# aleflabo/PREGO

Measured on AMD Instinct MI355X. Metric: frames/sec (per-frame action logits) on Assembly101-O TSN features, higher is better.
Workload: dtype fp16; 1 GPU; BASELINE configs[1]: Assembly101-O-test-split-shaped eval set, MiniROAD eval path (rgb+flow fp32 [T,2048] each -> per-frame probs[86] + argmax); clips_per_gpu=182, frames_per_gpu=2306143, min_T=3342, max_T=33981, flow=non-zero (full K=4096 layer1 GEMM), parallelism=clip-sharded dp1, no collective: every rank its own eval-set-sized clip list, weights=random init, seed 20

## Files before the change

prego_amd/csrc/ff_pass.hip:

```cpp
#include "common.h"
#include "kernels.h"
#include "pass_handshake.h"

#define FBK 64
#define FHALF 16384
#define FBUF 65536
#define FF_WAIT(n) asm volatile("s_waitcnt vmcnt(" #n ")" ::: "memory")
#define FF_TIMEOUT_TICKS 200000000ull

__device__ __forceinline__ int ffp_key_b(int r) { return ((r >> 1) & 1) | (((r >> 3) & 3) << 1); }

__device__ __forceinline__ bool ffp_wait_ge(const unsigned* p, unsigned need, unsigned* abort_word, unsigned code) {
  if (__hip_atomic_load(p, __ATOMIC_RELAXED, __HIP_MEMORY_SCOPE_AGENT) >= need) return true;
  const unsigned long long t0 = __builtin_amdgcn_s_memrealtime();
  unsigned spins = 0;
  for (;;) {
    __builtin_amdgcn_s_sleep(8);
    if (__hip_atomic_load(p, __ATOMIC_RELAXED, __HIP_MEMORY_SCOPE_AGENT) >= need) return true;
    if ((++spins & 31u) == 0u) {
      if (__hip_atomic_load(abort_word, __ATOMIC_RELAXED, __HIP_MEMORY_SCOPE_AGENT)) return false;
      if (__builtin_amdgcn_s_memrealtime() - t0 > FF_TIMEOUT_TICKS) {
        __hip_atomic_store(abort_word, code, __ATOMIC_RELAXED, __HIP_MEMORY_SCOPE_AGENT);
        return false;
      }
    }
  }
}

template <typename OT, bool SC1OUT>
__device__ __forceinline__ void ffp_tile(char* smem, const bf16_t* __restrict__ A, int lda, int rows, const bf16_t* __restrict__ B, int ldb,
                                         const float* __restrict__ bias, bf16_t* __restrict__ C, int ldc, int K) {
  int tid = threadIdx.x;
  asm volatile("" : "+v"(tid));
  const int lane = tid & 63;
  const int wave = __builtin_amdgcn_readfirstlane(tid >> 6);
  const int grp = wave >> 2, wc = wave & 3;
  const int nk = K / FBK;
  const int sr = lane >> 3, scp = lane & 7;
  int a_off[2], b_off[2];
#pragma unroll
  for (int i = 0; i < 2; ++i) {
    const int r = (wave * 2 + i) * 8 + sr;
    a_off[i] = r * lda * 2 + ((scp ^ ((r >> 1) & 7)) << 4);
    b_off[i] = r * ldb * 2 + ((scp ^ ffp_key_b(r)) << 4);
  }
  const __amdgpu_buffer_rsrc_t rs_a = __builtin_amdgcn_make_buffer_rsrc((void*)A, 0, rows * lda * 2, 0x00020000);
  const __amdgpu_buffer_rsrc_t rs_b = __builtin_amdgcn_make_buffer_rsrc((void*)B, 0, 256 * ldb * 2, 0x00020000);
  auto stage_a = [&](int hf, int kt) {
    char* dst = smem + (kt & 1) * FBUF + hf * FHALF + wave * 2048;
    const int so = hf * 128 * lda * 2 + kt * (FBK * 2);
#pragma unroll
    for (int i = 0; i < 2; ++i)
      __builtin_amdgcn_raw_ptr_buffer_load_lds(rs_a, (__attribute__((address_space(3))) void*)(dst + i * 1024), 16, a_off[i], so, 0, 0);
  };
  auto stage_b = [&](int hf, int kt) {
    char* dst = smem + (kt & 1) * FBUF + (2 + hf) * FHALF + wave * 2048;
    const int so = hf * 128 * ldb * 2 + kt * (FBK * 2);
#pragma unroll
    for (int i = 0; i < 2; ++i)
      __builtin_amdgcn_raw_ptr_buffer_load_lds(rs_b, (__attribute__((address_space(3))) void*)(dst + i * 1024), 16, b_off[i], so, 0, 0);
  };
  const int fr = lane & 15, fq = lane >> 4;
  bf16x8 a0[2][4], a1[2][4], b0[2][2], b1[2][2];
  auto read_a = [&](bf16x8 (&af)[2][4], int slot, int kt) {
    const char* base = smem + (kt & 1) * FBUF + slot * FHALF;
#pragma unroll
    for (int ks = 0; ks < 2; ++ks)
#pragma unroll
      for (int i = 0; i < 4; ++i) {
        const int r = grp * 64 + i * 16 + fr;
        af[ks][i] = *(const bf16x8*)(base + r * 128 + (((ks * 4 + fq) ^ ((r >> 1) & 7)) << 4));
      }
  };
  auto read_b = [&](bf16x8 (&bf)[2][2], int slot, int kt) {
    const char* base = smem + (kt & 1) * FBUF + slot * FHALF;
#pragma unroll
    for (int ks = 0; ks < 2; ++ks)
#pragma unroll
      for (int j = 0; j < 2; ++j) {
        const int r = wc * 32 + (fr >> 2) * 8 + j * 4 + (fr & 3);
        bf[ks][j] = *(const bf16x8*)(base + r * 128 + (((ks * 4 + fq) ^ ffp_key_b(r)) << 4));
      }
  };
  f32x4 acc[2][2][4][2];
#pragma unroll
  for (int x = 0; x < 2; ++x)
#pragma unroll
    for (int y = 0; y < 2; ++y)
#pragma unroll
      for (int i = 0; i < 4; ++i)
#pragma unroll
        for (int j = 0; j < 2; ++j) acc[x][y][i][j] = (f32x4){0.f, 0.f, 0.f, 0.f};
  auto mma = [&](f32x4 (&c)[4][2], const bf16x8 (&af)[2][4], const bf16x8 (&bf)[2][2]) {
    asm volatile("s_waitcnt lgkmcnt(0)" ::: "memory");
    __builtin_amdgcn_sched_barrier(0);
    __builtin_amdgcn_s_setprio(1);
#pragma unroll
    for (int ks = 0; ks < 2; ++ks)
#pragma unroll
      for (int i = 0; i < 4; ++i)
#pragma unroll
        for (int j = 0; j < 2; ++j) c[i][j] = op16<OT>::mfma(bf[ks][j], af[ks][i], c[i][j]);
    __builtin_amdgcn_s_setprio(0);
    __builtin_amdgcn_sched_barrier(0);
  };
  auto bar = [&]() {
    __builtin_amdgcn_sched_barrier(0);
    __builtin_amdgcn_s_barrier();
    __builtin_amdgcn_sched_barrier(0);
  };
  stage_a(0, 0); stage_b(0, 0); stage_b(1, 0); stage_a(1, 0);
  stage_a(0, 1); stage_b(0, 1); stage_b(1, 1);
  FF_WAIT(10);
  bar();
  read_a(a0, 0, 0);
  if (grp == 1) bar();
  for (int kt = 0; kt < nk; ++kt) {
    const bool full = kt + 2 < nk;
    read_b(b0, 2, kt);
    if (kt + 1 < nk) stage_a(1, kt + 1);
    if (full) FF_WAIT(10); else FF_WAIT(0);
    bar();
    mma(acc[0][0], a0, b0);
    bar();
    read_b(b1, 3, kt);
    if (full) { stage_a(0, kt + 2); FF_WAIT(10); } else FF_WAIT(0);
    bar();
    mma(acc[0][1], a0, b1);
    bar();
    read_a(a1, 1, kt);
    if (full) { stage_b(0, kt + 2); FF_WAIT(10); } else FF_WAIT(0);
    bar();
    mma(acc[1][1], a1, b1);
    bar();
    if (kt + 1 < nk) read_a(a0, 0, kt + 1);
    if (full) { stage_b(1, kt + 2); FF_WAIT(10); } else FF_WAIT(0);
    bar();
    mma(acc[1][0], a1, b0);
    bar();
  }
  if (grp == 0) bar();
  float4 bv[2][2];
#pragma unroll
  for (int y = 0; y < 2; ++y)
#pragma unroll
    for (int j = 0; j < 2; ++j) bv[y][j] = *(const float4*)(bias + y * 128 + wc * 32 + fq * 8 + j * 4);
  const __amdgpu_buffer_rsrc_t rs_c = __builtin_amdgcn_make_buffer_rsrc((void*)C, 0, rows * ldc * 2, 0x00020000);
#pragma unroll
  for (int x = 0; x < 2; ++x)
#pragma unroll
    for (int y = 0; y < 2; ++y) {
      const int n = y * 128 + wc * 32 + fq * 8;
#pragma unroll
      for (int i = 0; i < 4; ++i) {
        const int m = x * 128 + grp * 64 + i * 16 + fr;
        const f32x4 v0 = acc[x][y][i][0], v1 = acc[x][y][i][1];
        u32x4 pk;
        pk[0] = op16<OT>::pack2_sat(v0[0] + bv[y][0].x, v0[1] + bv[y][0].y); pk[1] = op16<OT>::pack2_sat(v0[2] + bv[y][0].z, v0[3] + bv[y][0].w);
        pk[2] = op16<OT>::pack2_sat(v1[0] + bv[y][1].x, v1[1] + bv[y][1].y); pk[3] = op16<OT>::pack2_sat(v1[2] + bv[y][1].z, v1[3] + bv[y][1].w);
        if constexpr (SC1OUT) __builtin_amdgcn_raw_buffer_store_b128(pk, rs_c, (m * ldc + n) * 2, 0, AUX_SC1);
        else __builtin_amdgcn_raw_buffer_store_b128(pk, rs_c, (m * ldc + n) * 2, 0, 0);
      }
    }
}

template <typename OT, bool IN16>
__device__ __forceinline__ void ffp_pack_rows(const FfPassArgs& a, int my_rows, int wave, int lane, const char* srgb, const char* sflow,
                                              bf16_t* __restrict__ Xs) {
  constexpr int ES = IN16 ? 2 : 4, NV = IN16 ? 1 : 2;
  constexpr int PR = 2;
  const int din = a.kx;
  const int cr_rgb = (a.d_rgb + 2047) >> 11, cpr = cr_rgb + ((a.d_flow + 2047) >> 11);
  const int n_rounds = my_rows > 0 ? ((my_rows + PR - 1) / PR) * cpr : 0;
  auto readlane_ptr = [](const char* p, int l) -> const char* {
    const unsigned long long v = (unsigned long long)p;
    const unsigned lo = (unsigned)__builtin_amdgcn_readlane((int)(unsigned)v, l), hi = (unsigned)__builtin_amdgcn_readlane((int)(unsigned)(v >> 32), l);
    return (const char*)(((unsigned long long)hi << 32) | lo);
  };
  int voff_in = lane * 8 * ES, voff_in2 = voff_in + 1024 * ES, voff_out = lane * 16;
  asm volatile("" : "+v"(voff_in), "+v"(voff_in2), "+v"(voff_out));
  auto issue = [&](u32x4 (&v)[PR][4][NV], int k) {
    const int rp = k / cpr, cj = k - rp * cpr;
    const bool fl = cj >= cr_rgb;
    const int cwin = (fl ? cj - cr_rgb : cj) << 11, seg_len = fl ? a.d_flow : a.d_rgb;
#pragma unroll
    for (int e = 0; e < PR; ++e) {
      const int r = rp * PR + e, rr = r < my_rows ? r : 0;
      const char* s0 = readlane_ptr(srgb, rr);
      const char* s1 = readlane_ptr(sflow, rr);
      const char* src = fl ? s1 : s0;
      const __amdgpu_buffer_rsrc_t rs = __builtin_amdgcn_make_buffer_rsrc((void*)(src + (size_t)cwin * ES), 0,
                                                                          (r < my_rows && src != nullptr) ? (seg_len - cwin) * ES : 0, 0x00020000);
#pragma unroll
      for (int b = 0; b < 4; ++b)
#pragma unroll
        for (int w = 0; w < NV; ++w)
          v[e][b][w] = __builtin_amdgcn_raw_buffer_load_b128(rs, (b < 2 ? voff_in : voff_in2) + ((b & 1) * 512 * ES + 16 * w), 0, AUX_NT);
    }
  };
  auto drain = [&](const u32x4 (&v)[PR][4][NV], int k) {
    const int rp = k / cpr, cj = k - rp * cpr;
    const bool fl = cj >= cr_rgb;
    const int cwin = (fl ? cj - cr_rgb : cj) << 11, seg_len = fl ? a.d_flow : a.d_rgb, seg_base = fl ? a.d_rgb : 0;
#pragma unroll
    for (int e = 0; e < PR; ++e) {
      const int r = rp * PR + e;
      bf16_t* dst = Xs + (size_t)(wave * 32 + (r < my_rows ? r : 0)) * din + seg_base + cwin;
      const __amdgpu_buffer_rsrc_t rs = __builtin_amdgcn_make_buffer_rsrc((void*)dst, 0, r < my_rows ? (seg_len - cwin) * 2 : 0, 0x00020000);
#pragma unroll
      for (int b = 0; b < 4; ++b) {
        u32x4 o = v[e][b][0];
        if constexpr (!IN16) {
          const u32x4 x = v[e][b][0], y = v[e][b][NV - 1];
          o[0] = op16<OT>::pack2_sat(__uint_as_float(x[0]), __uint_as_float(x[1])); o[1] = op16<OT>::pack2_sat(__uint_as_float(x[2]), __uint_as_float(x[3]));
          o[2] = op16<OT>::pack2_sat(__uint_as_float(y[0]), __uint_as_float(y[1])); o[3] = op16<OT>::pack2_sat(__uint_as_float(y[2]), __uint_as_float(y[3]));
        }
        __builtin_amdgcn_raw_buffer_store_b128(o, rs, voff_out + b * 1024, 0, 0);
      }
    }
  };
  u32x4 va[PR][4][NV], vb[PR][4][NV];
  if (n_rounds == 0) return;
  issue(va, 0);
  int k = 0;
#define PACK_FENCE() __builtin_amdgcn_sched_barrier(0)
  for (; k + 2 < n_rounds; k += 2) {
    issue(vb, k + 1); PACK_FENCE();
    drain(va, k); PACK_FENCE();
    issue(va, k + 2); PACK_FENCE();
    drain(vb, k + 1); PACK_FENCE();
  }
  if (k + 1 < n_rounds) {
    issue(vb, k + 1); PACK_FENCE();
    drain(va, k); PACK_FENCE();
    drain(vb, k + 1);
  } else {
    drain(va, k);
  }
#undef PACK_FENCE
}

template <typename OT>
__device__ __forceinline__ void ffp_pack(const FfPassArgs& a, int row0, int nrows, bf16_t* __restrict__ Xs) {
  int tid_ = threadIdx.x;
  asm volatile("" : "+v"(tid_));
  const int lane = tid_ & 63, wave = __builtin_amdgcn_readfirstlane(tid_ >> 6);
  const int rl = wave * 32 + (lane & 31);
  int clip = 0, t = 0;
  if (rl < nrows) {
    const int row = row0 + rl;
    int lo = a.plan.blk_step[row >> 5];
    while (lo + 1 < a.plan.s_max && a.plan.rowoff[lo + 1] <= row) ++lo;
    const int slot = row - a.plan.rowoff[lo];
    int k = a.plan.seg_off[slot];
    const int kend = a.plan.seg_off[slot + 1];
    while (k + 1 < kend && a.plan.seg_start[k + 1] <= lo) ++k;
    clip = a.plan.seg_clip[k];
    t = lo - a.plan.seg_start[k];
    if (a.rowmap != nullptr && lane < 32) ((int2*)a.rowmap)[row] = make_int2(clip, t);
  }
  const char* srgb = nullptr; const char* sflow = nullptr;
  const int es = a.in16 ? 2 : 4;
  if (rl < nrows) {
    const float* rgb = a.rgb_ptrs ? a.rgb_ptrs[clip] : nullptr;
    const float* flow = a.flow_ptrs ? a.flow_ptrs[clip] : nullptr;
    if (rgb) srgb = (const char*)rgb + (size_t)t * a.d_rgb * es;
    if (flow) sflow = (const char*)flow + (size_t)t * a.d_flow * es;
  }
  const int my_rows = nrows - wave * 32 < 32 ? nrows - wave * 32 : 32;
  if (a.in16) ffp_pack_rows<OT, true>(a, my_rows, wave, lane, srgb, sflow, Xs);
  else ffp_pack_rows<OT, false>(a, my_rows, wave, lane, srgb, sflow, Xs);
}

constexpr int FLN_MAX_E = 2048;

template <typename OT, int NV, int NR>
__device__ __forceinline__ void ffp_ln(const FfPassArgs& a, int nrows, const bf16_t* __restrict__ Ys, bf16_t* __restrict__ Es, const float* gb) {
  int tid_ = threadIdx.x;
  asm volatile("" : "+v"(tid_));
  const int lane = tid_ & 63, wave = __builtin_amdgcn_readfirstlane(tid_ >> 6);
  const int E = NV * 512;
  const float fE = (float)a.E;
  if (wave >= nrows) return;
  auto request = [&](u32x4 (&dst)[NR][NV], int rb) {
#pragma unroll
    for (int e = 0; e < NR; ++e) {
      int r = rb + 8 * e;
      if (r >= nrows) r = wave;
      const bf16_t* y = Ys + (size_t)r * E;
#pragma unroll
      for (int i = 0; i < NV; ++i) dst[e][i] = *(const u32x4*)(y + (i * 64 + lane) * 8);
    }
  };
  auto unpack = [](const u32x4 w, float (&f)[8]) {
    f[0] = op16<OT>::lo(w[0]); f[1] = op16<OT>::hi(w[0]); f[2] = op16<OT>::lo(w[1]); f[3] = op16<OT>::hi(w[1]);
    f[4] = op16<OT>::lo(w[2]); f[5] = op16<OT>::hi(w[2]); f[6] = op16<OT>::lo(w[3]); f[7] = op16<OT>::hi(w[3]);
  };
  auto process = [&](const u32x4 (&raw)[NR][NV], int rb) {
    float s[NR];
#pragma unroll
    for (int e = 0; e < NR; ++e) {
      s[e] = 0.f;
#pragma unroll
      for (int i = 0; i < NV; ++i) {
        float f[8];
        unpack(raw[e][i], f);
        s[e] += ((f[0] + f[1]) + (f[2] + f[3])) + ((f[4] + f[5]) + (f[6] + f[7]));
      }
    }
    auto wave_sum_rows = [](float (&v)[NR]) {
#pragma unroll
      for (int o = 32; o > 0; o >>= 1) {
        float t[NR];
#pragma unroll
        for (int e = 0; e < NR; ++e) t[e] = __shfl_xor(v[e], o, 64);
#pragma unroll
        for (int e = 0; e < NR; ++e) v[e] += t[e];
      }
    };
    float mu[NR], rstd[NR];
    wave_sum_rows(s);
#pragma unroll
    for (int e = 0; e < NR; ++e) mu[e] = s[e] / fE;
#pragma unroll
    for (int e = 0; e < NR; ++e) {
      float qq = 0.f;
#pragma unroll
      for (int i = 0; i < NV; ++i) {
        float f[8];
        unpack(raw[e][i], f);
#pragma unroll
        for (int k = 0; k < 8; ++k) {
#pragma clang fp contract(off)
          const float d = f[k] - mu[e];
          const float dd = d * d;
          qq = qq + dd;
        }
      }
      rstd[e] = qq;
    }
    wave_sum_rows(rstd);
#pragma unroll
    for (int e = 0; e < NR; ++e) rstd[e] = 1.0f / sqrtf(rstd[e] / fE + a.ln_eps);
#pragma unroll
    for (int i = 0; i < NV; ++i) {
      const int c = (i * 64 + lane) * 8;
      const float4 g0 = *(const float4*)(gb + c), g1 = *(const float4*)(gb + c + 4);
      const float4 b0 = *(const float4*)(gb + FLN_MAX_E + c), b1 = *(const float4*)(gb + FLN_MAX_E + c + 4);
      const float gg[8] = {g0.x, g0.y, g0.z, g0.w, g1.x, g1.y, g1.z, g1.w};
      const float bb[8] = {b0.x, b0.y, b0.z, b0.w, b1.x, b1.y, b1.z, b1.w};
#pragma unroll
      for (int e = 0; e < NR; ++e) {
        float f[8], o[8];
        unpack(raw[e][i], f);
#pragma unroll
        for (int k = 0; k < 8; ++k) o[k] = fmaxf((f[k] - mu[e]) * rstd[e] * gg[k] + bb[k], 0.f);
        uint4 w;
        w.x = op16<OT>::pack2_sat(o[0], o[1]); w.y = op16<OT>::pack2_sat(o[2], o[3]); w.z = op16<OT>::pack2_sat(o[4], o[5]); w.w = op16<OT>::pack2_sat(o[6], o[7]);
        if (rb + 8 * e < nrows) *(uint4*)(Es + (size_t)(rb + 8 * e) * E + c) = w;
      }
    }
  };
  constexpr int STEP = 8 * NR;
#define LN_FENCE() __builtin_amdgcn_sched_barrier(0)
  u32x4 ra[NR][NV], rbuf[NR][NV];
  int rb = wave;
  request(ra, rb); LN_FENCE();
  for (; rb + 2 * STEP < nrows; rb += 2 * STEP) {
    request(rbuf, rb + STEP); LN_FENCE();
    process(ra, rb); LN_FENCE();
    request(ra, rb + 2 * STEP); LN_FENCE();
    process(rbuf, rb + STEP); LN_FENCE();
  }
  if (rb + STEP < nrows) {
    request(rbuf, rb + STEP); LN_FENCE();
    process(ra, rb); LN_FENCE();
    process(rbuf, rb + STEP);
  } else {
    process(ra, rb);
  }
#undef LN_FENCE
}

template <typename OT, int MAXV, int NR>
__device__ __forceinline__ void ffp_ln_generic(const FfPassArgs& a, int nrows, const bf16_t* __restrict__ Ys, bf16_t* __restrict__ Es) {
  int tid_ = threadIdx.x;
  asm volatile("" : "+v"(tid_));
  const int lane = tid_ & 63, wave = tid_ >> 6;
  const int E = a.E, nv = E / 512;
  u32x4 raw[NR][MAXV], nxt[NR][MAXV];
  auto request = [&](u32x4 (&dst)[NR][MAXV], int rb) {
#pragma unroll
    for (int e = 0; e < NR; ++e) {
      int r = rb + 8 * e;
      if (r >= nrows) r = wave < nrows ? wave : 0;
      const bf16_t* y = Ys + (size_t)r * E;
#pragma unroll
      for (int i = 0; i < MAXV; ++i)
        if (i < nv) dst[e][i] = *(const u32x4*)(y + (i * 64 + lane) * 8);
    }
  };
  if (wave < nrows) request(raw, wave);
  for (int rb = wave; rb < nrows; rb += 8 * NR) {
    if (rb + 8 * NR < nrows) request(nxt, rb + 8 * NR);
    auto unpack = [](const u32x4 w, float (&f)[8]) {
      f[0] = op16<OT>::lo(w[0]); f[1] = op16<OT>::hi(w[0]); f[2] = op16<OT>::lo(w[1]); f[3] = op16<OT>::hi(w[1]);
      f[4] = op16<OT>::lo(w[2]); f[5] = op16<OT>::hi(w[2]); f[6] = op16<OT>::lo(w[3]); f[7] = op16<OT>::hi(w[3]);
    };
    float s[NR];
#pragma unroll
    for (int e = 0; e < NR; ++e) {
      s[e] = 0.f;
#pragma unroll
      for (int i = 0; i < MAXV; ++i)
        if (i < nv) {
          float f[8];
          unpack(raw[e][i], f);
          s[e] += ((f[0] + f[1]) + (f[2] + f[3])) + ((f[4] + f[5]) + (f[6] + f[7]));
        }
    }
    float mu[NR], rstd[NR];
#pragma unroll
    for (int e = 0; e < NR; ++e) mu[e] = wave_sum(s[e]) / (float)E;
#pragma unroll
    for (int e = 0; e < NR; ++e) {
      float qq = 0.f;
#pragma unroll
      for (int i = 0; i < MAXV; ++i)
        if (i < nv) {
          float f[8];
          unpack(raw[e][i], f);
#pragma unroll
          for (int k = 0; k < 8; ++k) {
#pragma clang fp contract(off)
            const float d = f[k] - mu[e];
            const float dd = d * d;
            qq = qq + dd;
          }
        }
      rstd[e] = qq;
    }
#pragma unroll
    for (int e = 0; e < NR; ++e) rstd[e] = 1.0f / sqrtf(wave_sum(rstd[e]) / (float)E + a.ln_eps);
#pragma unroll
    for (int i = 0; i < MAXV; ++i)
      if (i < nv) {
        const int c = (i * 64 + lane) * 8;
        const float4 g0 = *(const float4*)(a.ln_g + c), g1 = *(const float4*)(a.ln_g + c + 4);
        const float4 b0 = *(const float4*)(a.ln_b + c), b1 = *(const float4*)(a.ln_b + c + 4);
        const float gg[8] = {g0.x, g0.y, g0.z, g0.w, g1.x, g1.y, g1.z, g1.w};
        const float bb[8] = {b0.x, b0.y, b0.z, b0.w, b1.x, b1.y, b1.z, b1.w};
#pragma unroll
        for (int e = 0; e < NR; ++e) {
          float f[8], o[8];
          unpack(raw[e][i], f);
#pragma unroll
          for (int k = 0; k < 8; ++k) o[k] = fmaxf((f[k] - mu[e]) * rstd[e] * gg[k] + bb[k], 0.f);
          uint4 w;
          w.x = op16<OT>::pack2_sat(o[0], o[1]); w.y = op16<OT>::pack2_sat(o[2], o[3]); w.z = op16<OT>::pack2_sat(o[4], o[5]); w.w = op16<OT>::pack2_sat(o[6], o[7]);
          if (rb + 8 * e < nrows) *(uint4*)(Es + (size_t)(rb + 8 * e) * E + c) = w;
        }
      }
    if (rb + 8 * NR < nrows) {
#pragma unroll
      for (int e = 0; e < NR; ++e)
#pragma unroll
        for (int i = 0; i < MAXV; ++i)
          if (i < nv) raw[e][i] = nxt[e][i];
    }
  }
}

template <typename OT>
__device__ __forceinline__ void ffp_ln_any(const FfPassArgs& a, int nrows, const bf16_t* __restrict__ Ys, bf16_t* __restrict__ Es, const float* gb) {
  switch (a.E >> 9) {
    case 4: ffp_ln<OT, 4, 2>(a, nrows, Ys, Es, gb); break;
    case 2: ffp_ln<OT, 2, 4>(a, nrows, Ys, Es, gb); break;
    case 1: ffp_ln<OT, 1, 4>(a, nrows, Ys, Es, gb); break;
    default: ffp_ln_generic<OT, 8, 2>(a, nrows, Ys, Es); break;
  }
}

template <typename OT>
__global__ __launch_bounds__(512, 2) void ff_pass_kernel(FfPassArgs a) {
  extern __shared__ __attribute__((aligned(16))) char smem[];
  __shared__ int s_job[2];
  const int tid = threadIdx.x;
  const int xcc = __builtin_amdgcn_readfirstlane(__builtin_amdgcn_s_getreg((3 << 11) | 20) & 7);
  if (xcc < a.xcd_lo) return;
  if (tid == 0) {
    const unsigned nth = __hip_atomic_fetch_add(a.hs.ff_here + xcc, 1u, __ATOMIC_RELAXED, __HIP_MEMORY_SCOPE_AGENT);
    s_job[1] = hs_wait(a.hs, a.hs.ticks_all) == PREGO_HS_GO ? 1 : 0;
    if (a.max_wg > 0 && (int)nth >= a.max_wg) s_job[1] = 0;
  }
  __syncthreads();
  if (!__builtin_amdgcn_readfirstlane(s_job[1])) return;
  __shared__ __attribute__((aligned(16))) float s_gb[2 * FLN_MAX_E];
  if (a.E <= FLN_MAX_E)
    for (int c = tid; c < a.E; c += 512) { s_gb[c] = a.ln_g[c]; s_gb[FLN_MAX_E + c] = a.ln_b[c]; }
  const int q = xcc - a.xcd_lo, nf = 8 - a.xcd_lo;
  const int n_q = a.n_units > q ? (a.n_units - q + nf - 1) / nf : 0;
  const int sg = a.sg, tpr = sg * (2 + a.nt1 + a.nt2);
  const int n_rounds = (n_q + sg - 1) / sg + a.lag3;
  __shared__ unsigned long long s_stat[11];
  const bool stats = a.stats != nullptr && tid == 0;
  if (stats) {
    for (int e = 0; e < 8; ++e) s_stat[e] = 0;
    s_stat[9] = __builtin_amdgcn_s_memrealtime(); s_stat[8] = s_stat[9]; s_stat[10] = __builtin_amdgcn_s_memtime();
  }
#define FSTAT(i) do { if (stats) { const unsigned long long n_ = __builtin_amdgcn_s_memrealtime(); s_stat[i] += n_ - s_stat[8]; s_stat[8] = n_; } } while (0)
  for (;;) {
    __syncthreads();
    if (tid == 0) s_job[0] = (int)__hip_atomic_fetch_add(a.tick + q, 1u, __ATOMIC_RELAXED, __HIP_MEMORY_SCOPE_AGENT);
    __syncthreads();
    const int k = __builtin_amdgcn_readfirstlane(s_job[0]);
    const int round = k / tpr, j = k - round * tpr;
    FSTAT(5);
    if (round >= n_rounds) break;
    int type, i, nb = 0;
    if (j < sg) { type = 0; i = round * sg + j; }
    else if (j < sg + sg * a.nt1) { const int jj = j - sg; type = 1; nb = jj / sg; i = (round - a.lag1) * sg + (jj - nb * sg); }
    else if (j < 2 * sg + sg * a.nt1) { type = 2; i = (round - a.lag2) * sg + (j - sg - sg * a.nt1); }
    else { const int jj = j - 2 * sg - sg * a.nt1; type = 3; nb = jj / sg; i = (round - a.lag3) * sg + (jj - nb * sg); }
    if (i < 0 || i >= n_q) continue;
    const int u = q + i * nf;
    if (tid == 0) {
      bool ok = true;
      const int up = u - a.ring_units;
      if (type == 0) {
        if (up >= 0) ok = ffp_wait_ge(a.l1_cnt + up, (unsigned)a.nt1, a.abort_word, 0x100u);
      } else if (type == 1) {
        ok = ffp_wait_ge(a.pack_done + u, 1u, a.abort_word, 0x101u);
        if (ok && up >= 0) ok = ffp_wait_ge(a.ln_done + up, 1u, a.abort_word, 0x102u);
      } else if (type == 2) {
        ok = ffp_wait_ge(a.l1_cnt + u, (unsigned)a.nt1, a.abort_word, 0x103u);
        if (ok && up >= 0) ok = ffp_wait_ge(a.wih_cnt + up, (unsigned)a.nt2, a.abort_word, 0x104u);
      } else {
        ok = ffp_wait_ge(a.ln_done + u, 1u, a.abort_word, 0x105u);
        const int ug = u - a.gi_ring_units;
        if (ok && ug >= 0) ok = ffp_wait_ge(a.rec_cnt + (ug >> a.chunk_unit_shift), (unsigned)a.rec_expect, a.abort_word, 0x106u);
      }
      s_job[1] = ok ? 1 : 0;
    }
    __syncthreads();
    if (!__builtin_amdgcn_readfirstlane(s_job[1])) break;
    FSTAT(4);
    asm volatile("buffer_inv sc0" ::: "memory");
    const int row0 = u * 256;
    const int nrows = a.total_rows - row0 < 256 ? a.total_rows - row0 : 256;
    const size_t slot = (size_t)(u % a.ring_units) * 256;
    if (type == 0) {
      if (!(a.dbg & 1)) ffp_pack<OT>(a, row0, nrows, a.X + slot * a.kx);
    } else if (type == 1) {
      if (!(a.dbg & 4))
      ffp_tile<OT, false>(smem, a.X + slot * a.kx, a.kx, nrows, a.w1 + (size_t)nb * 256 * a.ld_w1, a.ld_w1, a.b1 + nb * 256,
                          a.Y + slot * a.E + nb * 256, a.E, a.kx);
    } else if (type == 2) {
      if (a.dbg & 2) { }
      else ffp_ln_any<OT>(a, nrows, a.Y + slot * a.E, a.Eb + slot * a.E, s_gb);
    } else {
      const size_t gslot = (size_t)(u & (a.gi_ring_units - 1)) * 256;
      if (!(a.dbg & 8))
      ffp_tile<OT, true>(smem, a.Eb + slot * a.E, a.E, nrows, a.w_ih + (size_t)nb * 256 * a.E, a.E, a.bias2 + nb * 256,
                         a.GI + gslot * a.n3 + nb * 256, a.n3, a.E);
    }
    asm volatile("s_waitcnt vmcnt(0)" ::: "memory");
    __syncthreads();
    FSTAT(type);
    if (tid == 0) {
      if (type == 0) __hip_atomic_store(a.pack_done + u, 1u, __ATOMIC_RELAXED, __HIP_MEMORY_SCOPE_AGENT);
      else if (type == 1) __hip_atomic_fetch_add(a.l1_cnt + u, 1u, __ATOMIC_RELAXED, __HIP_MEMORY_SCOPE_AGENT);
      else if (type == 2) __hip_atomic_store(a.ln_done + u, 1u, __ATOMIC_RELAXED, __HIP_MEMORY_SCOPE_AGENT);
      else {
        const unsigned old = __hip_atomic_fetch_add(a.wih_cnt + u, 1u, __ATOMIC_RELAXED, __HIP_MEMORY_SCOPE_AGENT);
        if (old + 1u == (unsigned)a.nt2)
          __hip_atomic_fetch_add(a.gi_cnt + (u >> a.chunk_unit_shift), 1u, __ATOMIC_RELAXED, __HIP_MEMORY_SCOPE_AGENT);
      }
    }
  }
  if (stats) {
    s_stat[7] = __builtin_amdgcn_s_memrealtime() - s_stat[9];
    s_stat[6] = __builtin_amdgcn_s_memtime() - s_stat[10];
    for (int e = 0; e < 8; ++e) atomicAdd(a.stats + e, s_stat[e]);
  }
#undef FSTAT
}

int launch_ff_pass(const FfPassArgs& a, hipStream_t s) {
  if (a.E % 512 || a.E > 4096 || a.kx % FBK || a.kx < 2 * FBK || a.n3 % 256 || a.xcd_lo < 1 || a.xcd_lo > 7) return -1;
  if (a.sg < 1 || a.ring_units % (8 - a.xcd_lo) || (a.gi_ring_units & (a.gi_ring_units - 1)) || a.nt1 != a.E / 256 || a.nt2 != a.n3 / 256) return -1;
  static DeviceOnce once;
  once.run([&] {
    (void)hipFuncSetAttribute((const void*)ff_pass_kernel<bf16_t>, hipFuncAttributeMaxDynamicSharedMemorySize, 2 * FBUF);
    (void)hipFuncSetAttribute((const void*)ff_pass_kernel<f16_t>, hipFuncAttributeMaxDynamicSharedMemorySize, 2 * FBUF);
  });
  if (a.f16) ff_pass_kernel<f16_t><<<256, 512, 2 * FBUF, s>>>(a);
  else ff_pass_kernel<bf16_t><<<256, 512, 2 * FBUF, s>>>(a);
  return 0;
}
```

Baseline: 23.57 million frames/s.

## Prefetch next GEMM tile's first K-stages during current tile's epilogue

```diff
diff --git a/prego_amd/csrc/ff_pass.hip b/prego_amd/csrc/ff_pass.hip
--- a/prego_amd/csrc/ff_pass.hip
+++ b/prego_amd/csrc/ff_pass.hip
@@ -27,9 +27,37 @@
   }
 }
 
-template <typename OT, bool SC1OUT>
+__device__ __forceinline__ void ffp_first_stages(char* smem, const bf16_t* __restrict__ A, int lda, int rows, const bf16_t* __restrict__ B, int ldb) {
+  int tid = threadIdx.x;
+  asm volatile("" : "+v"(tid));
+  const int lane = tid & 63;
+  const int wave = __builtin_amdgcn_readfirstlane(tid >> 6);
+  const int sr = lane >> 3, scp = lane & 7;
+  const __amdgpu_buffer_rsrc_t rs_a = __builtin_amdgcn_make_buffer_rsrc((void*)A, 0, rows * lda * 2, 0x00020000);
+  const __amdgpu_buffer_rsrc_t rs_b = __builtin_amdgcn_make_buffer_rsrc((void*)B, 0, 256 * ldb * 2, 0x00020000);
+#pragma unroll
+  for (int kt = 0; kt < 2; ++kt)
+#pragma unroll
+    for (int s = 0; s < 4; ++s) {
+      if (kt == 1 && s == 3) break;
+      const bool is_a = s == 0 || s == 3;
+      const int hf = s == 0 ? 0 : s == 3 ? 1 : s - 1;
+      const int ld = is_a ? lda : ldb;
+      char* dst = smem + kt * FBUF + (is_a ? hf : 2 + hf) * FHALF + wave * 2048;
+      const int so = hf * 128 * ld * 2 + kt * (FBK * 2);
+#pragma unroll
+      for (int i = 0; i < 2; ++i) {
+        const int r = (wave * 2 + i) * 8 + sr;
+        const int off = r * ld * 2 + ((scp ^ (is_a ? ((r >> 1) & 7) : ffp_key_b(r))) << 4);
+        __builtin_amdgcn_raw_ptr_buffer_load_lds(is_a ? rs_a : rs_b, (__attribute__((address_space(3))) void*)(dst + i * 1024), 16, off, so, 0, 0);
+      }
+    }
+}
+
+template <typename OT, bool SC1OUT, typename Ahead>
 __device__ __forceinline__ void ffp_tile(char* smem, const bf16_t* __restrict__ A, int lda, int rows, const bf16_t* __restrict__ B, int ldb,
-                                         const float* __restrict__ bias, bf16_t* __restrict__ C, int ldc, int K) {
+                                         const float* __restrict__ bias, bf16_t* __restrict__ C, int ldc, int K, bool staged, const Ahead& ah,
+                                         int* s_job, int& next_k, bool& next_staged) {
   int tid = threadIdx.x;
   asm volatile("" : "+v"(tid));
   const int lane = tid & 63;
@@ -109,42 +137,56 @@
     __builtin_amdgcn_s_barrier();
     __builtin_amdgcn_sched_barrier(0);
   };
-  stage_a(0, 0); stage_b(0, 0); stage_b(1, 0); stage_a(1, 0);
-  stage_a(0, 1); stage_b(0, 1); stage_b(1, 1);
+  if (!staged) ffp_first_stages(smem, A, lda, rows, B, ldb);
   FF_WAIT(10);
   bar();
   read_a(a0, 0, 0);
   if (grp == 1) bar();
-  for (int kt = 0; kt < nk; ++kt) {
-    const bool full = kt + 2 < nk;
+  unsigned tk = 0, p0 = 0, p1 = 0;
+  auto kstep = [&](int kt, auto last_c) {
+    constexpr int LAST = decltype(last_c)::value;
     read_b(b0, 2, kt);
-    if (kt + 1 < nk) stage_a(1, kt + 1);
-    if (full) FF_WAIT(10); else FF_WAIT(0);
+    if (LAST < 2) stage_a(1, kt + 1);
+    if (LAST == 0) FF_WAIT(10); else if (LAST == 1) FF_WAIT(0);
     bar();
     mma(acc[0][0], a0, b0);
     bar();
+    if (LAST == 1 && tid == 0) tk = ah.draw();
+    if (LAST == 2 && tid == 0) ah.probe(__builtin_amdgcn_readfirstlane(tk), p0, p1);
     read_b(b1, 3, kt);
-    if (full) { stage_a(0, kt + 2); FF_WAIT(10); } else FF_WAIT(0);
+    if (LAST == 0) { stage_a(0, kt + 2); FF_WAIT(10); }
     bar();
     mma(acc[0][1], a0, b1);
     bar();
     read_a(a1, 1, kt);
-    if (full) { stage_b(0, kt + 2); FF_WAIT(10); } else FF_WAIT(0);
+    if (LAST == 0) { stage_b(0, kt + 2); FF_WAIT(10); }
     bar();
     mma(acc[1][1], a1, b1);
     bar();
-    if (kt + 1 < nk) read_a(a0, 0, kt + 1);
-    if (full) { stage_b(1, kt + 2); FF_WAIT(10); } else FF_WAIT(0);
+    if (LAST < 2) read_a(a0, 0, kt + 1);
+    if (LAST == 0) { stage_b(1, kt + 2); FF_WAIT(10); }
     bar();
     mma(acc[1][0], a1, b0);
     bar();
-  }
+  };
+  for (int kt = 0; kt + 2 < nk; ++kt) kstep(kt, std::integral_constant<int, 0>{});
+  kstep(nk - 2, std::integral_constant<int, 1>{});
+  kstep(nk - 1, std::integral_constant<int, 2>{});
   if (grp == 0) bar();
-  float4 bv[2][2];
+  f32x4 bv[2][2];
 #pragma unroll
   for (int y = 0; y < 2; ++y)
 #pragma unroll
-    for (int j = 0; j < 2; ++j) bv[y][j] = *(const float4*)(bias + y * 128 + wc * 32 + fq * 8 + j * 4);
+    for (int j = 0; j < 2; ++j) bv[y][j] = *(const f32x4*)(bias + y * 128 + wc * 32 + fq * 8 + j * 4);
+#pragma unroll
+  for (int y = 0; y < 2; ++y)
+#pragma unroll
+    for (int j = 0; j < 2; ++j) asm volatile("" : "+v"(bv[y][j]));
+  if (tid == 0) s_job[1] = (s_job[4] && p0 >= (unsigned)s_job[2] && p1 >= (unsigned)s_job[3]) ? 1 : 0;
+  __syncthreads();
+  next_k = __builtin_amdgcn_readfirstlane(s_job[0]);
+  next_staged = __builtin_amdgcn_readfirstlane(s_job[1]) != 0;
+  if (next_staged) ah.stage(next_k);
   const __amdgpu_buffer_rsrc_t rs_c = __builtin_amdgcn_make_buffer_rsrc((void*)C, 0, rows * ldc * 2, 0x00020000);
 #pragma unroll
   for (int x = 0; x < 2; ++x)
@@ -156,8 +198,8 @@
         const int m = x * 128 + grp * 64 + i * 16 + fr;
         const f32x4 v0 = acc[x][y][i][0], v1 = acc[x][y][i][1];
         u32x4 pk;
-        pk[0] = op16<OT>::pack2_sat(v0[0] + bv[y][0].x, v0[1] + bv[y][0].y); pk[1] = op16<OT>::pack2_sat(v0[2] + bv[y][0].z, v0[3] + bv[y][0].w);
-        pk[2] = op16<OT>::pack2_sat(v1[0] + bv[y][1].x, v1[1] + bv[y][1].y); pk[3] = op16<OT>::pack2_sat(v1[2] + bv[y][1].z, v1[3] + bv[y][1].w);
+        pk[0] = op16<OT>::pack2_sat(v0[0] + bv[y][0][0], v0[1] + bv[y][0][1]); pk[1] = op16<OT>::pack2_sat(v0[2] + bv[y][0][2], v0[3] + bv[y][0][3]);
+        pk[2] = op16<OT>::pack2_sat(v1[0] + bv[y][1][0], v1[1] + bv[y][1][1]); pk[3] = op16<OT>::pack2_sat(v1[2] + bv[y][1][2], v1[3] + bv[y][1][3]);
         if constexpr (SC1OUT) __builtin_amdgcn_raw_buffer_store_b128(pk, rs_c, (m * ldc + n) * 2, 0, AUX_SC1);
         else __builtin_amdgcn_raw_buffer_store_b128(pk, rs_c, (m * ldc + n) * 2, 0, 0);
       }
@@ -481,10 +523,60 @@
   }
 }
 
+__device__ __forceinline__ void ffp_decode(const FfPassArgs& a, int k, int tpr, int& round, int& type, int& i, int& nb) {
+  const int sg = a.sg;
+  round = k / tpr;
+  const int j = k - round * tpr;
+  nb = 0;
+  if (j < sg) { type = 0; i = round * sg + j; }
+  else if (j < sg + sg * a.nt1) { const int jj = j - sg; type = 1; nb = jj / sg; i = (round - a.lag1) * sg + (jj - nb * sg); }
+  else if (j < 2 * sg + sg * a.nt1) { type = 2; i = (round - a.lag2) * sg + (j - sg - sg * a.nt1); }
+  else { const int jj = j - 2 * sg - sg * a.nt1; type = 3; nb = jj / sg; i = (round - a.lag3) * sg + (jj - nb * sg); }
+}
+
+struct FfpAhead {
+  const FfPassArgs& a;
+  char* smem; int* s_job;
+  int q, nf, n_q, tpr, n_rounds;
+  __device__ __forceinline__ unsigned draw() const {
+    unsigned lim = 0xffffffffu;
+    asm volatile("" : "+v"(lim));
+    return __builtin_amdgcn_atomic_inc32((unsigned*)(a.tick + q), lim, __ATOMIC_RELAXED, "agent");
+  }
+  __device__ __forceinline__ void probe(int t, unsigned& p0, unsigned& p1) const {
+    int round, type, i, nb;
+    ffp_decode(a, t, tpr, round, type, i, nb);
+    const int u = q + i * nf, up = u - a.ring_units, ug = u - a.gi_ring_units;
+    const bool tile = round < n_rounds && i >= 0 && i < n_q && (type == 1 || type == 3);
+    const unsigned* w0 = a.tick + q; const unsigned* w1 = w0;
+    unsigned n0 = 0, n1 = 0;
+    if (tile && type == 1) {
+      w0 = a.pack_done + u; n0 = 1u;
+      if (up >= 0) { w1 = a.ln_done + up; n1 = 1u; }
+    } else if (tile) {
+      w0 = a.ln_done + u; n0 = 1u;
+      if (ug >= 0) { w1 = a.rec_cnt + (ug >> a.chunk_unit_shift); n1 = (unsigned)a.rec_expect; }
+    }
+    s_job[0] = t; s_job[2] = (int)n0; s_job[3] = (int)n1; s_job[4] = tile ? 1 : 0;
+    p0 = __hip_atomic_load(w0, __ATOMIC_RELAXED, __HIP_MEMORY_SCOPE_AGENT);
+    p1 = __hip_atomic_load(w1, __ATOMIC_RELAXED, __HIP_MEMORY_SCOPE_AGENT);
+  }
+  __device__ __forceinline__ void stage(int k) const {
+    int round, type, i, nb;
+    ffp_decode(a, k, tpr, round, type, i, nb);
+    const int u = q + i * nf;
+    const int nrows = a.total_rows - u * 256 < 256 ? a.total_rows - u * 256 : 256;
+    const size_t slot = (size_t)(u % a.ring_units) * 256;
+    asm volatile("buffer_inv sc0" ::: "memory");
+    if (type == 1) ffp_first_stages(smem, a.X + slot * a.kx, a.kx, nrows, a.w1 + (size_t)nb * 256 * a.ld_w1, a.ld_w1);
+    else ffp_first_stages(smem, a.Eb + slot * a.E, a.E, nrows, a.w_ih + (size_t)nb * 256 * a.E, a.E);
+  }
+};
+
 template <typename OT>
 __global__ __launch_bounds__(512, 2) void ff_pass_kernel(FfPassArgs a) {
   extern __shared__ __attribute__((aligned(16))) char smem[];
-  __shared__ int s_job[2];
+  __shared__ int s_job[5];
   const int tid = threadIdx.x;
   const int xcc = __builtin_amdgcn_readfirstlane(__builtin_amdgcn_s_getreg((3 << 11) | 20) & 7);
   if (xcc < a.xcd_lo) return;
@@ -500,8 +592,8 @@
     for (int c = tid; c < a.E; c += 512) { s_gb[c] = a.ln_g[c]; s_gb[FLN_MAX_E + c] = a.ln_b[c]; }
   const int q = xcc - a.xcd_lo, nf = 8 - a.xcd_lo;
   const int n_q = a.n_units > q ? (a.n_units - q + nf - 1) / nf : 0;
-  const int sg = a.sg, tpr = sg * (2 + a.nt1 + a.nt2);
-  const int n_rounds = (n_q + sg - 1) / sg + a.lag3;
+  const int tpr = a.sg * (2 + a.nt1 + a.nt2);
+  const int n_rounds = (n_q + a.sg - 1) / a.sg + a.lag3;
   __shared__ unsigned long long s_stat[11];
   const bool stats = a.stats != nullptr && tid == 0;
   if (stats) {
@@ -509,43 +601,49 @@
     s_stat[9] = __builtin_amdgcn_s_memrealtime(); s_stat[8] = s_stat[9]; s_stat[10] = __builtin_amdgcn_s_memtime();
   }
 #define FSTAT(i) do { if (stats) { const unsigned long long n_ = __builtin_amdgcn_s_memrealtime(); s_stat[i] += n_ - s_stat[8]; s_stat[8] = n_; } } while (0)
+  const FfpAhead ah{a, smem, s_job, q, nf, n_q, tpr, n_rounds};
+  int k = -1;
+  bool staged = false;
   for (;;) {
-    __syncthreads();
-    if (tid == 0) s_job[0] = (int)__hip_atomic_fetch_add(a.tick + q, 1u, __ATOMIC_RELAXED, __HIP_MEMORY_SCOPE_AGENT);
-    __syncthreads();
-    const int k = __builtin_amdgcn_readfirstlane(s_job[0]);
-    const int round = k / tpr, j = k - round * tpr;
-    FSTAT(5);
+    if (k < 0) {
+      __syncthreads();
+      if (tid == 0) s_job[0] = (int)__hip_atomic_fetch_add(a.tick + q, 1u, __ATOMIC_RELAXED, __HIP_MEMORY_SCOPE_AGENT);
+      __syncthreads();
+      k = __builtin_amdgcn_readfirstlane(s_job[0]);
+      FSTAT(5);
+    }
+    int round, type, i, nb;
+    ffp_decode(a, k, tpr, round, type, i, nb);
+    k = -1;
     if (round >= n_rounds) break;
-    int type, i, nb = 0;
-    if (j < sg) { type = 0; i = round * sg + j; }
-    else if (j < sg + sg * a.nt1) { const int jj = j - sg; type = 1; nb = jj / sg; i = (round - a.lag1) * sg + (jj - nb * sg); }
-    else if (j < 2 * sg + sg * a.nt1) { type = 2; i = (round - a.lag2) * sg + (j - sg - sg * a.nt1); }
-    else { const int jj = j - 2 * sg - sg * a.nt1; type = 3; nb = jj / sg; i = (round - a.lag3) * sg + (jj - nb * sg); }
     if (i < 0 || i >= n_q) continue;
     const int u = q + i * nf;
-    if (tid == 0) {
-      bool ok = true;
-      const int up = u - a.ring_units;
-      if (type == 0) {
-        if (up >= 0) ok = ffp_wait_ge(a.l1_cnt + up, (unsigned)a.nt1, a.abort_word, 0x100u);
-      } else if (type == 1) {
-        ok = ffp_wait_ge(a.pack_done + u, 1u, a.abort_word, 0x101u);
-        if (ok && up >= 0) ok = ffp_wait_ge(a.ln_done + up, 1u, a.abort_word, 0x102u);
-      } else if (type == 2) {
-        ok = ffp_wait_ge(a.l1_cnt + u, (unsigned)a.nt1, a.abort_word, 0x103u);
-        if (ok && up >= 0) ok = ffp_wait_ge(a.wih_cnt + up, (unsigned)a.nt2, a.abort_word, 0x104u);
-      } else {
-        ok = ffp_wait_ge(a.ln_done + u, 1u, a.abort_word, 0x105u);
-        const int ug = u - a.gi_ring_units;
-        if (ok && ug >= 0) ok = ffp_wait_ge(a.rec_cnt + (ug >> a.chunk_unit_shift), (unsigned)a.rec_expect, a.abort_word, 0x106u);
-      }
-      s_job[1] = ok ? 1 : 0;
-    }
-    __syncthreads();
-    if (!__builtin_amdgcn_readfirstlane(s_job[1])) break;
-    FSTAT(4);
-    asm volatile("buffer_inv sc0" ::: "memory");
+    const bool was_staged = staged;
+    staged = false;
+    if (!was_staged) {
+      if (tid == 0) {
+        bool ok = true;
+        const int up = u - a.ring_units;
+        if (type == 0) {
+          if (up >= 0) ok = ffp_wait_ge(a.l1_cnt + up, (unsigned)a.nt1, a.abort_word, 0x100u);
+        } else if (type == 1) {
+          ok = ffp_wait_ge(a.pack_done + u, 1u, a.abort_word, 0x101u);
+          if (ok && up >= 0) ok = ffp_wait_ge(a.ln_done + up, 1u, a.abort_word, 0x102u);
+        } else if (type == 2) {
+          ok = ffp_wait_ge(a.l1_cnt + u, (unsigned)a.nt1, a.abort_word, 0x103u);
+          if (ok && up >= 0) ok = ffp_wait_ge(a.wih_cnt + up, (unsigned)a.nt2, a.abort_word, 0x104u);
+        } else {
+          ok = ffp_wait_ge(a.ln_done + u, 1u, a.abort_word, 0x105u);
+          const int ug = u - a.gi_ring_units;
+          if (ok && ug >= 0) ok = ffp_wait_ge(a.rec_cnt + (ug >> a.chunk_unit_shift), (unsigned)a.rec_expect, a.abort_word, 0x106u);
+        }
+        s_job[1] = ok ? 1 : 0;
+      }
+      __syncthreads();
+      if (!__builtin_amdgcn_readfirstlane(s_job[1])) break;
+      FSTAT(4);
+      asm volatile("buffer_inv sc0" ::: "memory");
+    }
     const int row0 = u * 256;
     const int nrows = a.total_rows - row0 < 256 ? a.total_rows - row0 : 256;
     const size_t slot = (size_t)(u % a.ring_units) * 256;
@@ -554,7 +652,7 @@
     } else if (type == 1) {
       if (!(a.dbg & 4))
       ffp_tile<OT, false>(smem, a.X + slot * a.kx, a.kx, nrows, a.w1 + (size_t)nb * 256 * a.ld_w1, a.ld_w1, a.b1 + nb * 256,
-                          a.Y + slot * a.E + nb * 256, a.E, a.kx);
+                          a.Y + slot * a.E + nb * 256, a.E, a.kx, was_staged, ah, s_job, k, staged);
     } else if (type == 2) {
       if (a.dbg & 2) { }
       else ffp_ln_any<OT>(a, nrows, a.Y + slot * a.E, a.Eb + slot * a.E, s_gb);
@@ -562,7 +660,7 @@
       const size_t gslot = (size_t)(u & (a.gi_ring_units - 1)) * 256;
       if (!(a.dbg & 8))
       ffp_tile<OT, true>(smem, a.Eb + slot * a.E, a.E, nrows, a.w_ih + (size_t)nb * 256 * a.E, a.E, a.bias2 + nb * 256,
-                         a.GI + gslot * a.n3 + nb * 256, a.n3, a.E);
+                         a.GI + gslot * a.n3 + nb * 256, a.n3, a.E, was_staged, ah, s_job, k, staged);
     }
     asm volatile("s_waitcnt vmcnt(0)" ::: "memory");
     __syncthreads();
```

Result: no change. 23.80 million frames/s (median of 6 runs) (+1.0%).
